# chngdickson/ov2slam

Hardware: AMD Instinct MI355X
Metric: tracked_frames_per_sec (higher is better)
Workload: dtype u8/s16 fixed-point + f32

## Files before the change

### include/ov2slam_hip.h

```cpp
#ifndef OV2SLAM_HIP_H
#define OV2SLAM_HIP_H

#include <stddef.h>
#include <stdint.h>

#ifdef __cplusplus
extern "C" {
#endif

typedef int ov2_status;
enum {
    OV2_OK = 0,
    OV2_ERR_INVALID = -1,
    OV2_ERR_HIP = -2,
    OV2_ERR_NOMEM = -3,
    OV2_ERR_NODEVICE = -4,
    OV2_ERR_UNSUPPORTED = -5
};

typedef struct ov2_ctx ov2_ctx;
typedef struct ov2_images ov2_images;
typedef struct ov2_pyr ov2_pyr;

ov2_status ov2_ctx_create(int device, ov2_ctx **out);
// ... 47 lines not shown
void ov2_pyr_release(ov2_pyr *p);
void ov2_pyr_release_from(ov2_ctx *user, ov2_pyr *p);
int ov2_pyr_batch(const ov2_pyr *p);
int ov2_pyr_nlevels(const ov2_pyr *p);
ov2_status ov2_pyr_level_size(const ov2_pyr *p, int level, int *w, int *h, int *pad);
ov2_status ov2_pyr_download_level(ov2_ctx *ctx, const ov2_pyr *p, int b, int level, uint8_t *img, int16_t *grad);

ov2_status ov2_klt_track_fb(ov2_ctx *ctx, const ov2_pyr *prev, const ov2_pyr *cur, int win, int nlevels,
                            int max_iter, float eps, float err_th, float fb_th, int n, const float *kps_xy,
                            float *priors_xy, uint8_t *status);
ov2_status ov2_klt_track_fb_dev(ov2_ctx *ctx, const ov2_pyr *prev, const ov2_pyr *cur, int win, int nlevels,
                                int max_iter, float eps, float err_th, float fb_th, int n, const float *d_kps_xy,
                                float *d_priors_xy, uint8_t *d_status, const int32_t *d_img_idx,
                                uint32_t *d_iters);

ov2_status ov2_klt_tracking_frame_dev(ov2_ctx *ctx, const ov2_pyr *prev, const ov2_pyr *cur, int win,
                                      int nlevels_full, int max_iter, float eps, float err_th, float fb_th, int n,
                                      const float *d_kps_xy, const float *d_prior_xy, const uint8_t *d_has_prior,
                                      const int32_t *d_img_idx, float *d_out_xy, uint8_t *d_out_status,
                                      int32_t *d_p3p_req , uint32_t *d_iters );

ov2_status ov2_klt_set_lanes(ov2_ctx *ctx, int lanes);
ov2_status ov2_klt_set_stereo_split(ov2_ctx *ctx, int k);

ov2_status ov2_line_min_sad(ov2_ctx *ctx, const ov2_pyr *left, const ov2_pyr *right, int level, int nwinsize, int go_left,
                            int n, const float *pts_xy, float *xprior, float *l1err);
ov2_status ov2_line_min_sad_dev(ov2_ctx *ctx, const ov2_pyr *left, const ov2_pyr *right, int level, int nwinsize,
                                int go_left, int n, const float *d_pts_xy, const int32_t *d_img_idx, float *d_xprior,
                                float *d_l1err);

typedef struct ov2_cam_model {
    double K[4];
    int32_t model;
    int32_t n_coeffs;
    double D[5];
} ov2_cam_model;

ov2_status ov2_stereo_matching(ov2_ctx *ctx, const ov2_pyr *left, const ov2_pyr *right, int win, int nlevels_full,
                               int max_iter, float eps, float err_th, float fb_th, int n, const float *kps_xy,
                               const float *prior_xy, const uint8_t *has_prior, const float *lunpx_xy, int rectified,
                               const double *F_rl, const ov2_cam_model *right_cam, float *out_rxy, uint8_t *out_status);
ov2_status ov2_stereo_matching_dev(ov2_ctx *ctx, const ov2_pyr *left, const ov2_pyr *right, int win, int nlevels_full,
                                   int max_iter, float eps, float err_th, float fb_th, int n, const float *d_kps_xy,
                                   const float *d_prior_xy, const uint8_t *d_has_prior, const int32_t *d_img_idx,
                                   const float *d_lunpx_xy, int rectified, const double *F_rl, const ov2_cam_model *right_cam,
                                   float *d_out_rxy, uint8_t *d_out_status, uint32_t *d_iters);
// ... 487 lines not shown
```

### ov2slam_amd/_lib.py

```python
import ctypes as C
import os

_HERE = os.path.dirname(os.path.abspath(__file__))
LIB_PATH = os.environ.get("OV2SLAM_HIP_LIB") or os.path.join(_HERE, "lib", "libov2hip.so")

vp = C.c_void_p
vpp = C.POINTER(C.c_void_p)
ip = C.POINTER(C.c_int)
fp = C.POINTER(C.c_float)

SIGNATURES = {
    "ov2_ctx_create": (C.c_int, [C.c_int, vpp]),
    "ov2_ctx_create_ex": (C.c_int, [C.c_int, C.c_int, vpp]),
    "ov2_ctx_destroy": (None, [vp]),
    "ov2_last_error": (C.c_char_p, [vp]),
    "ov2_status_string": (C.c_char_p, [C.c_int]),
    "ov2_ctx_synchronize": (C.c_int, [vp]),
    "ov2_ctx_set_kf_overlap": (C.c_int, [vp, C.c_int]),
    "ov2_ctx_set_kf_lazy_join": (C.c_int, [vp, C.c_int]),
    "ov2_ctx_get_kf_lazy_join": (C.c_int, [vp]),
    "ov2_ctx_kf_join_stats": (C.c_int, [vp, C.POINTER(C.c_int64)]),
    "ov2_kf_ranges_independent": (C.c_int, [C.POINTER(C.c_size_t), C.c_int, C.POINTER(C.c_size_t), C.c_int,
                                            C.POINTER(C.c_size_t), C.c_int, C.POINTER(C.c_size_t), C.c_int]),
    "ov2_ctx_set_wave_prio": (C.c_int, [vp, C.c_int]),
# ... 17 lines not shown
    "ov2_memcpy_d2h": (C.c_int, [vp, vp, vp, C.c_size_t]),
    "ov2_memcpy_d2d": (C.c_int, [vp, vp, vp, C.c_size_t]),
    "ov2_images_create": (C.c_int, [vp, C.c_int, C.c_int, C.c_int, vpp]),
    "ov2_images_upload": (C.c_int, [vp, vp, C.c_int, vp, C.c_int]),
    "ov2_images_destroy": (None, [vp]),
    "ov2_pyramid_build": (C.c_int, [vp, vp, C.c_int, C.c_int, C.c_int, C.c_int, C.c_int, C.c_int, C.c_float,
                                    C.c_int, C.c_int, vpp]),
    "ov2_pyramid_build_images": (C.c_int, [vp, vp, C.c_int, C.c_int, C.c_int, C.c_float, C.c_int, C.c_int, vpp]),
    "ov2_pyr_retain": (None, [vp]),
    "ov2_pyr_release": (None, [vp]),
    "ov2_pyr_release_from": (None, [vp, vp]),
    "ov2_pyr_batch": (C.c_int, [vp]),
    "ov2_pyr_nlevels": (C.c_int, [vp]),
    "ov2_pyr_level_size": (C.c_int, [vp, C.c_int, ip, ip, ip]),
    "ov2_pyr_download_level": (C.c_int, [vp, vp, C.c_int, C.c_int, vp, vp]),
    "ov2_klt_track_fb": (C.c_int, [vp, vp, vp, C.c_int, C.c_int, C.c_int, C.c_float, C.c_float, C.c_float,
                                   C.c_int, vp, vp, vp]),
    "ov2_klt_track_fb_dev": (C.c_int, [vp, vp, vp, C.c_int, C.c_int, C.c_int, C.c_float, C.c_float, C.c_float,
                                       C.c_int, vp, vp, vp, vp, vp]),
    "ov2_klt_tracking_frame_dev": (C.c_int, [vp, vp, vp, C.c_int, C.c_int, C.c_int, C.c_float, C.c_float,
                                             C.c_float, C.c_int, vp, vp, vp, vp, vp, vp, vp, vp]),
    "ov2_klt_set_lanes": (C.c_int, [vp, C.c_int]),
    "ov2_klt_set_stereo_split": (C.c_int, [vp, C.c_int]),
    "ov2_line_min_sad": (C.c_int, [vp, vp, vp, C.c_int, C.c_int, C.c_int, C.c_int, vp, vp, vp]),
    "ov2_line_min_sad_dev": (C.c_int, [vp, vp, vp, C.c_int, C.c_int, C.c_int, C.c_int, vp, vp, vp, vp]),
    "ov2_stereo_matching": (C.c_int, [vp, vp, vp, C.c_int, C.c_int, C.c_int, C.c_float, C.c_float, C.c_float, C.c_int,
                                      vp, vp, vp, vp, C.c_int, vp, vp, vp, vp]),
    "ov2_stereo_matching_dev": (C.c_int, [vp, vp, vp, C.c_int, C.c_int, C.c_int, C.c_float, C.c_float, C.c_float, C.c_int,
                                          vp, vp, vp, vp, vp, C.c_int, vp, vp, vp, vp, vp]),
    "ov2_detect_grid": (C.c_int, [vp, vp, C.c_int, C.c_int, C.c_int, C.POINTER(C.c_double), C.c_int, vp, vp, C.c_int, ip, vp]),
    "ov2_detect_grid_batch": (C.c_int, [vp, vp, C.c_int, C.c_int, C.POINTER(C.c_double), ip, vp, vp, C.c_int, ip, vp, C.c_int]),
    "ov2_detect_grid_batch_dev": (C.c_int, [vp, vp, C.c_int, C.c_int, vp, C.c_int, vp, vp, vp, vp, C.c_int, vp, vp, C.c_int]),
    "ov2_fast_detect_batch": (C.c_int, [vp, vp, C.c_int, C.c_int, vp, vp, C.c_int, C.c_int, vp, vp, vp, vp]),
    "ov2_fast_detect_batch_dev": (C.c_int, [vp, vp, C.c_int, C.c_int, C.c_int, vp, vp, C.c_int, C.c_int, vp, vp, vp, vp]),
    "ov2_ba_default_options": (None, [vp, C.c_float]),
    "ov2_ba_solve": (C.c_int, [vp, vp, vp, vp]),
    "ov2_ba_solve_batch": (C.c_int, [vp, C.c_int, vp, vp, vp]),
    "ov2_ba_solve_batch_dev": (C.c_int, [vp, C.c_int, vp, vp, vp]),
    "ov2_pnp_solve_batch_dev": (C.c_int, [vp, C.c_int, vp, vp, vp, vp, vp, vp, C.c_int, C.c_float, C.c_int, C.c_int,
                                          vp, vp, vp, vp]),
    "ov2_map_create": (C.c_int, [vp, C.c_int, C.c_int, C.c_int, vp]),
    "ov2_map_destroy": (None, [vp]),
    "ov2_map_add_keyframe": (C.c_int, [vp, C.c_int, vp, C.c_int, vp, vp, vp, vp, vp]),
    "ov2_map_set_landmarks": (C.c_int, [vp, C.c_int, vp, vp, vp]),
    "ov2_map_set_poses": (C.c_int, [vp, C.c_int, vp, vp]),
    "ov2_map_remove_obs": (C.c_int, [vp, C.c_int, vp, vp]),
# ... 103 lines not shown
```

### ov2slam_amd/csrc/ctx.hip

```cpp
#include "ov2_internal.h"

#include <cstdlib>

ov2_status ov2_set_err(ov2_ctx *ctx, ov2_status s, const char *fmt, ...)
{
    char buf[512];
    va_list ap;
    va_start(ap, fmt);
    vsnprintf(buf, sizeof(buf), fmt, ap);
    va_end(ap);
    if (ctx) {
        std::lock_guard<std::mutex> g(ctx->mu);
        ctx->err = buf;
    }
    return s;
}

extern "C" const char *ov2_status_string(ov2_status s)
{
    switch (s) {
    case OV2_OK: return "ok";
    case OV2_ERR_INVALID: return "invalid argument";
    case OV2_ERR_HIP: return "HIP runtime error";
    case OV2_ERR_NOMEM: return "out of memory";
// ... 91 lines not shown
    if (device < 0 || device >= ndev) return OV2_ERR_INVALID;
    if (hipSetDevice(device) != hipSuccess) return OV2_ERR_HIP;
    uint32_t mask[MAX_MASK_WORDS];
    int mask_words = 0, effective_cus = 0;
    if (n_cus > 0) {
        const int total = device_cus(device);
        if (n_cus >= total || total > 32 * MAX_MASK_WORDS || ov2_cu_mask_build(total, n_cus, layout, mask) != OV2_OK) return OV2_ERR_INVALID;
        mask_words = (total + 31) / 32;
        for (int x = 0; x < OV2_CU_MASK_XCDS; ++x) {
            int bits = 0, own = 0;
            for (int k = x; k < total; k += OV2_CU_MASK_XCDS, ++own) bits += (int)(mask[k >> 5] >> (k & 31) & 1u);
            effective_cus += bits ? bits : own;
        }
    }
    ov2_ctx *c = new ov2_ctx();
    c->device = device;
    c->scratch_dev = nullptr;
    c->scratch_bytes = 0;
    c->tmp_img = nullptr;
    c->ktime_on = false;
    c->wave_prio = high_priority ? OV2_WAVE_PRIO_HIGH : 0;
    c->klt_lanes = 0;
    c->klt_stereo_split = -1;
    c->knn_lanes = 0;
    c->knn_cus = effective_cus;
    c->cu_share = n_cus;
    c->cu_layout = layout;
    c->counts_as_high = false;
    c->lcd_splits = 0;
    c->lcd_calls = 0;
    c->ba_arena = nullptr;
    c->ba_arena_cap = 0;
    c->ba_host = nullptr;
    c->ba_host_cap = 0;
    c->ba_copy_stream = nullptr;
    c->klt_counts[0] = c->klt_counts[1] = nullptr;
    c->klt_counts_words = 0;
    c->klt_counts_cur = 0;
    c->klt_counts_dirty = true;
    c->ba_copy_ev[0] = c->ba_copy_ev[1] = nullptr;
    c->ba_arena2 = nullptr;
    c->ba_arena2_cap = 0;
    c->stage_host = c->stage_dev = nullptr;
    c->stage_cap = 0;
    c->stage_ev = nullptr;
    c->stage_ev_pending = false;
// ... 506 lines not shown
```

### ov2slam_amd/csrc/klt.hip

```cpp
#include <cstdlib>

#include "ov2_internal.h"
#include "ov2_wave.h"

using namespace ov2wave;

namespace {

struct klt_params {
    int win, nlevels, max_iter;
    int wave_prio;
    double eps2;
    float err_th;
    double fb_th;
    float min_eig_thr;
    int rule33;
};

#define W_BITS 14

__device__ __forceinline__ void lk_weights(float a, float b, int &w00, int &w01, int &w10, int &w11)
{
    w00 = (int)__builtin_rintf((1.f - a) * (1.f - b) * (float)(1 << W_BITS));
    w01 = (int)__builtin_rintf(a * (1.f - b) * (float)(1 << W_BITS));
// ... 110 lines not shown
    asm("v_ashrrev_i32_sdwa %0, %2, %1 dst_sel:WORD_1 dst_unused:UNUSED_PRESERVE src0_sel:DWORD src1_sel:DWORD" : "+v"(keep) : "v"(acc), "n"(SH));
    return keep;
}

struct level_ptrs {
    const unsigned char *img;
    const int *grad;
    int istride, gstride, w, h, rows;
    const unsigned char *base;
    unsigned img_o, grad_o;
};

__device__ __forceinline__ level_ptrs level_of(const ov2_pyr_view &v, int l, int b)
{
    level_ptrs p;
    const ov2_level_desc &L = v.lv[l];
    p.img = v.base + L.img_off + L.img_bstride * b;
    p.grad = reinterpret_cast<const int *>(v.base + L.grad_off + L.grad_bstride * b);
    p.istride = L.istride; p.gstride = L.gstride; p.w = L.w; p.h = L.h; p.rows = L.rows;
    p.base = v.base; p.img_o = (unsigned)(L.img_off + L.img_bstride * b); p.grad_o = (unsigned)(L.grad_off + L.grad_bstride * b);
    return p;
}

template <int WIN, int GL>
__device__ __forceinline__ int lk_level(const level_ptrs &I, const level_ptrs &J, int pad, int level, int max_level,
                                        bool run, float kx, float ky, float &nx_io, float &ny_io, int &status,
                                        float &err, const klt_params &P, int sub, unsigned &passes,
                                        unsigned char *lwI, unsigned char *lwJ, unsigned char *lg)
{
    constexpr int GROW = klt_lds<WIN>::GSEG * 4;
    constexpr int OC = WIN < GL ? WIN : GL;
    constexpr int NE = (WIN - OC) * WIN;
    constexpr int NR = (NE + GL - 1) / GL;
    constexpr int NRP = (NR + 1) / 2;
    constexpr int NP = (WIN + 1) / 2;
    const float FLT_SCALE = 1.f / (float)(1 << 20);
    const float half = (float)(WIN - 1) * 0.5f;
    const float lscale = __builtin_ldexpf(1.f, -level);
    float px = kx * lscale, py = ky * lscale;
    float nx, ny;
    if (level == max_level) { nx = nx_io * lscale; ny = ny_io * lscale; }
    else { nx = nx_io * 2.f; ny = ny_io * 2.f; }
    if (run) { nx_io = nx; ny_io = ny; }

    px -= half; py -= half;
    const int ipx = (int)floorf(px), ipy = (int)floorf(py);
    if (run && (ipx < -WIN || ipx >= I.w || ipy < -WIN || ipy >= I.h)) {
        if (level == 0) { status = 0; err = 0.f; }
        run = false;
    }
    if (!__any(run)) return 0;
    if (run) passes += 1u;
    int w00, w01, w10, w11;
    lk_weights(px - (float)ipx, py - (float)ipy, w00, w01, w10, w11);

    const bool col = sub < OC;
    const int sc = col ? sub : 0;
    unsigned Iv2[NP], Ix2[NP], Iy2[NP];
    unsigned IvE[NRP > 0 ? NRP : 1], IxE[NRP > 0 ? NRP : 1], IyE[NRP > 0 ? NRP : 1];
    int eoff[NR > 0 ? NR : 1];
    int sA11 = 0, sA12 = 0, sA22 = 0;
    {
        const unsigned W01 = pack_lo16((unsigned)w00, (unsigned)w01), W23 = pack_lo16((unsigned)w10, (unsigned)w11);
        const int bx0 = run ? (OV2_LM + ipx) : OV2_LM, by = run ? (ipy + pad) : pad;
        {
            const float sx = nx - half, sy = ny - half;
            const int inx0 = (int)floorf(sx), iny0 = (int)floorf(sy);
            const bool in0 = run && !(inx0 < -WIN || inx0 >= J.w || iny0 < -WIN || iny0 >= J.h);
            __syncthreads();
            const int jx0 = OV2_LM + (in0 ? inx0 : 0);
            stage_u8<WIN, GL>(I.img + (size_t)by * I.istride + (bx0 & ~3), I.istride, lwI, sub);
            stage_grad<WIN, GL>(I.grad + (size_t)by * I.gstride + bx0, I.gstride, lg, sub);
            stage_u8<WIN, GL>(J.img + (size_t)((in0 ? iny0 : 0) + pad) * J.istride + (jx0 & ~3), J.istride, lwJ, sub);
            __syncthreads();
        }
        const lds_col ci = lds_col_of(lwI, (bx0 & 3) + sc);
        const int *gp = reinterpret_cast<const int *>(lg) + sc;
        unsigned T = spread_u8x2(lds_pair(ci, 0));
        unsigned GX, GY;
        {
            const unsigned g0 = (unsigned)gp[0], g1 = (unsigned)gp[1];
            GX = pack_lo16(g0, g1); GY = pack_hi16(g0, g1);
        }
        const bool on = run && col;
        unsigned piv = 0, pix = 0, piy = 0;
#pragma unroll
        for (int y = 0; y < WIN; ++y) {
            gp += GROW;
            const unsigned B = spread_u8x2(lds_pair(ci, y + 1));
            const unsigned h0 = (unsigned)gp[0], h1 = (unsigned)gp[1];
            const unsigned HX = pack_lo16(h0, h1), HY = pack_hi16(h0, h1);
            const unsigned iv = (unsigned)dot2(B, W23, dot2k(T, W01, 1 << (W_BITS - 5 - 1))) >> (W_BITS - 5);
            int ix = dot2(HX, W23, dot2k(GX, W01, 1 << (W_BITS - 1))) >> W_BITS;
            int iy = dot2(HY, W23, dot2k(GY, W01, 1 << (W_BITS - 1))) >> W_BITS;
            if (y & 1) {
                Iv2[y >> 1] = pack_lo16(piv, iv); Ix2[y >> 1] = pack_lo16(pix, (unsigned)ix); Iy2[y >> 1] = pack_lo16(piy, (unsigned)iy);
            } else if (y == WIN - 1) {
                Iv2[y >> 1] = iv; Ix2[y >> 1] = (unsigned)ix & 0xffffu; Iy2[y >> 1] = (unsigned)iy & 0xffffu;
            } else {
                piv = iv; pix = (unsigned)ix; piy = (unsigned)iy;
            }
            T = B; GX = HX; GY = HY;
        }
        {
            const unsigned onm = on ? 0xffffffffu : 0u;
#pragma unroll
            for (int q = 0; q < NP; ++q) {
                Ix2[q] &= onm; Iy2[q] &= onm;
                sA11 = dot2(Ix2[q], Ix2[q], sA11); sA12 = dot2(Ix2[q], Iy2[q], sA12); sA22 = dot2(Iy2[q], Iy2[q], sA22);
            }
        }
#pragma unroll
        for (int r = 0; r < NR; ++r) {
            const int e = sub + GL * r;
            const bool ev = e < NE;
            const int ec = ev ? e : 0;
            const int ecol = OC + ec / WIN, erow = ec - (ec / WIN) * WIN;
            eoff[r] = erow * 16 + ecol;
            const lds_col ce = lds_col_of(lwI + erow * 16, (bx0 & 3) + ecol);
            const int *gpe = reinterpret_cast<const int *>(lg) + erow * GROW + ecol;
            const unsigned T0 = spread_u8x2(lds_pair(ce, 0)), T1 = spread_u8x2(lds_pair(ce, 1));
            const unsigned g0 = (unsigned)gpe[0], g1 = (unsigned)gpe[1];
            const unsigned h0 = (unsigned)gpe[GROW], h1 = (unsigned)gpe[GROW + 1];
            const unsigned iv = (unsigned)dot2(T1, W23, dot2k(T0, W01, 1 << (W_BITS - 5 - 1))) >> (W_BITS - 5);
            int ix = dot2(pack_lo16(h0, h1), W23, dot2k(pack_lo16(g0, g1), W01, 1 << (W_BITS - 1))) >> W_BITS;
// ... 122 lines not shown

template <int GL>
struct klt_map {
    static constexpr int KPW = 64 / GL;
    static __device__ __forceinline__ int slot(int tid) { return tid / GL; }
    static __device__ __forceinline__ int sub(int tid) { return tid & (GL - 1); }
    static __device__ __forceinline__ bool lane_ok(int) { return true; }
};
template <>
struct klt_map<3> {
    static constexpr int KPW = 21;
    static __device__ __forceinline__ int slot(int tid) { return min((tid * 171) >> 9, KPW - 1); }
    static __device__ __forceinline__ int sub(int tid) { return tid == 63 ? 0 : tid - 3 * ((tid * 171) >> 9); }
    static __device__ __forceinline__ bool lane_ok(int tid) { return tid != 63; }
};

template <int WIN, int GL>
struct klt_smem {
    static constexpr int BYTES = (64 / GL) * (2 * klt_lds<WIN>::WB + klt_lds<WIN>::GB);
};
template <int WIN>
struct klt_smem<WIN, 3> {
    static constexpr int BYTES = klt_map<3>::KPW * klt3::RSZ;
};

__device__ __forceinline__ int sum3_i32(int v, int c)
{
    const int t1 = v + dpp_i32<0x138>(v);
    const int t = v + dpp_i32<0x138>(t1);
    const int u1 = dpp_mov_i32<0x130>(t), u2 = dpp_mov_i32<0x130>(u1);
    return c == 2 ? t : (c == 1 ? u1 : u2);
}
__device__ __forceinline__ double sum3_f64(double v, int c)
{
    const double s1 = dpp_f64<0x138>(v), s2 = dpp_f64<0x138>(s1);
    const double t = (v + s1) + s2;
    const double u1 = dpp_f64<0x130>(t), u2 = dpp_f64<0x130>(u1);
    return c == 2 ? t : (c == 1 ? u1 : u2);
}

__device__ __forceinline__ unsigned klt3_pair_sel(unsigned k) { return 0x0c010c00u + k * 0x00010001u; }

__device__ __forceinline__ void klt3_region_origin(const level_ptrs &J, int pad, int inx, int iny, int &rr0, int &cc0)
{
    rr0 = min(max(iny + pad - klt3::ROW_MARGIN, 0), J.rows - klt3::RROWS);
    cc0 = min(max((OV2_LM + inx - klt3::COL_LEAD) & ~(klt3::COL_ALIGN - 1), 0), J.istride - klt3::RBYTES);
// ... 251 lines not shown
            b1 = (float)sum3_i32(pb1, c) * FLT_SCALE;
            b2 = (float)sum3_i32(pb2, c) * FLT_SCALE;
        } else {
            b1 = (float)sum3_f64((double)pb1, c) * FLT_SCALE;
            b2 = (float)sum3_f64((double)pb2, c) * FLT_SCALE;
        }
        const float dx = (A12 * b2 - A22 * b1) * D;
        const float dy = (A12 * b1 - A11 * b2) * D;
        if (run) {
            ++iters;
            nx += dx; ny += dy;
            nx_io = nx + half; ny_io = ny + half;
            if ((double)dx * dx + (double)dy * dy <= P.eps2) run = false;
            else if (j > 0 && fabsf(dx + pdx) <= 0.01f && fabsf(dy + pdy) <= 0.01f) {
                nx_io -= dx * 0.5f; ny_io -= dy * 0.5f;
                run = false;
            }
            pdx = dx; pdy = dy;
        }
    }
    return iters;
}

template <int WIN, int GL>
__device__ __forceinline__ int lk_pass(const level_ptrs &I, const level_ptrs &J, int pad, int level, int max_level, bool run,
                                       float kx, float ky, float &nx_io, float &ny_io, int &status, float &err,
                                       const klt_params &P, int sub, bool lane_ok, unsigned &passes, unsigned char *smem, int slot)
{
    if constexpr (GL == 3) {
        return lk_level3<WIN>(I, J, pad, level, max_level, run, kx, ky, nx_io, ny_io, status, err, P, sub, lane_ok, passes,
                              smem + slot * klt3::RSZ);
    } else {
        constexpr int KPW = 64 / GL, WB = klt_lds<WIN>::WB, GB = klt_lds<WIN>::GB;
        return lk_level<WIN, GL>(I, J, pad, level, max_level, run, kx, ky, nx_io, ny_io, status, err, P, sub, passes,
                                 smem + slot * WB, smem + KPW * WB + slot * WB, smem + 2 * KPW * WB + slot * GB);
    }
}

struct __attribute__((aligned(16))) klt_handover { float fx, fy, err; unsigned work; };

template <int WIN, int GL>
__device__ __forceinline__ int fb_track(const ov2_pyr_view &pv, const ov2_pyr_view &cv, int b, bool act, float kx,
                                          float ky, float &fx, float &fy, const klt_params &P, int nlevels, int sub,
                                          bool lane_ok, unsigned &work, unsigned char *smem, int slot,
                                          int l_hi, int l_lo, float err0, unsigned work0, float &err_out)
{
    int status = 1;
    float err = err0;
    unsigned it = work0 & 0xffffu, passes = work0 >> 16;
    for (int l = l_hi; l >= l_lo; --l) {
        const level_ptrs I = level_of(pv, l, b), J = level_of(cv, l, b);
        it += lk_pass<WIN, GL>(I, J, pv.pad, l, nlevels, act, kx, ky, fx, fy, status, err, P, sub, lane_ok, passes, smem, slot);
    }
    if (l_lo > 0) {
        work = it | (passes << 16);
        err_out = err;
        return 0;
    }
    const int W0 = cv.lv[0].w, H0 = cv.lv[0].h;
    int ok = act && status && !(err > P.err_th) &&
             (1.f <= fx && fx < (float)W0 - 1.f && 1.f <= fy && fy < (float)H0 - 1.f);
    int st2 = 1;
    float e2 = 0.f, bx = kx, by = ky;
    {
        const level_ptrs I = level_of(cv, 0, b), J = level_of(pv, 0, b);
        it += lk_pass<WIN, GL>(I, J, cv.pad, 0, 0, ok != 0, fx, fy, bx, by, st2, e2, P, sub, lane_ok, passes, smem, slot);
    }
    if (ok) {
        if (!st2) ok = 0;
        else {
            const float dx = kx - bx, dy = ky - by;
            const double nrm = __dsqrt_rn((double)dx * dx + (double)dy * dy);
            if (nrm > P.fb_th) ok = 0;
        }
    }
    work = it | (passes << 16);
    return ok;
}

template <int WIN, int GL>
__device__ __forceinline__ int fb_track(const ov2_pyr_view &pv, const ov2_pyr_view &cv, int b, bool act, float kx,
                                          float ky, float &fx, float &fy, const klt_params &P, int nlevels, int sub,
                                          bool lane_ok, unsigned &work, unsigned char *smem, int slot)
{
    float err;
    return fb_track<WIN, GL>(pv, cv, b, act, kx, ky, fx, fy, P, nlevels, sub, lane_ok, work, smem, slot, nlevels, 0, 0.f, 0u, err);
}

#define KLT_GL8_MIN_KPS 65536
// ... 133 lines not shown
    const int total = is_a ? total_a : total_b;
    if (g * KLT_KPW >= total) return;
    ov2wave::set_wave_prio(P.wave_prio);
    const int slot = M::slot((int)threadIdx.x), sub = M::sub((int)threadIdx.x), idx = g * KLT_KPW + slot;
    const bool lane_ok = M::lane_ok((int)threadIdx.x);
    const bool act = idx < total && lane_ok;
    const int i = (is_a ? list_a : list_b)[idx < total ? idx : total - 1];
    const float2 kp = kps[i];
    const int b = img_idx ? img_idx[i] : 0;
    float2 pr = (is_a || !P.rule33) ? prior[i] : kp;
    unsigned work = 0;
    const int nl = is_a ? min(1, pv.nlevels - 1) : P.nlevels;
    const bool upper = SPLIT && !is_a;
    float err;
    const int ok = fb_track<WIN, KLT_GL>(pv, cv, b, act, kp.x, kp.y, pr.x, pr.y, P, nl, sub, lane_ok, work, smem, slot, nl,
                                         upper ? split_k + 1 : 0, 0.f, 0u, err);
    if (upper) {
        if (act && sub == 0) hand[i] = klt_handover{pr.x, pr.y, err, work};
        return;
    }
    klt_stage1_finish(act && sub == 0, is_a, i, b, n, ok, pr, work, out_xy, out_status, counts, iters, cnt, list_c);
}

template <int WIN, int KLT_GL>
__global__ __launch_bounds__(64) __attribute__((amdgpu_waves_per_eu(KLT_WAVES(WIN, KLT_GL)))) void klt_stage2_kernel(ov2_pyr_view pv, ov2_pyr_view cv, klt_params P, int n,
                                                        const float2 *__restrict__ kps,
                                                        const int *__restrict__ img_idx, float2 *__restrict__ out_xy,
                                                        unsigned char *__restrict__ out_status,
                                                        const unsigned *__restrict__ counts, int *__restrict__ p3p_req,
                                                        unsigned *__restrict__ iters, const int *__restrict__ list_c,
                                                        const unsigned *__restrict__ cnt, int batch,
                                                        unsigned *__restrict__ next_counts, int next_words,
                                                        const int *__restrict__ list_b, int b_word,
                                                        const float2 *__restrict__ prior,
                                                        int split_k ,
                                                        const klt_handover *__restrict__ hand)
{
    __shared__ __attribute__((aligned(16))) unsigned char smem[klt_smem<WIN, KLT_GL>::BYTES];
    using M = klt_map<KLT_GL>;
    constexpr int KLT_KPW = M::KPW;
    const int slot = M::slot((int)threadIdx.x), sub = M::sub((int)threadIdx.x);
    const bool lane_ok = M::lane_ok((int)threadIdx.x);
    for (int q = blockIdx.x * 64 + threadIdx.x; q < next_words; q += gridDim.x * 64) next_counts[q] = 0u;
    auto tally = [&](int b, int &n3, int &good) {
        n3 = 0; good = 0;
        if constexpr (KLT_GL == 3) {
            for (int q = sub; q < 64; q += 3) {
                const unsigned cw = counts[64 * b + q];
                n3 += (int)(cw & 0xffffu); good += (int)(cw >> 16);
            }
            n3 = sum3_i32(n3, sub); good = sum3_i32(good, sub);
        } else {
            for (int q = 0; q < 64 / KLT_GL; ++q) {
                const unsigned cw = counts[64 * b + sub * (64 / KLT_GL) + q];
                n3 += (int)(cw & 0xffffu); good += (int)(cw >> 16);
            }
            n3 = row_sum_i32<KLT_GL>(n3); good = row_sum_i32<KLT_GL>(good);
        }
    };
    if (p3p_req && P.rule33) {
        for (int b0 = blockIdx.x * KLT_KPW; b0 < batch; b0 += gridDim.x * KLT_KPW) {
            const int b = b0 + slot;
            int n3, good;
            tally(min(b, batch - 1), n3, good);
            if (b < batch && lane_ok && sub == 0 && n3 > 0 && (double)good < 0.33 * (double)n3) p3p_req[b] = 1;
        }
    }
    const int total_b = (int)cnt[b_word], total_c = (int)cnt[2];
    const bool b_first = split_k < 0 || !KLT_SPLIT_C_FIRST;
    const int groups_1 = ((b_first ? total_b : total_c) + KLT_KPW - 1) / KLT_KPW;
    const bool first = (int)blockIdx.x < groups_1;
    const bool is_b = first == b_first;
    const int g = first ? (int)blockIdx.x : (int)blockIdx.x - groups_1;
    const int total = is_b ? total_b : total_c;
    if (g * KLT_KPW >= total) return;
    ov2wave::set_wave_prio(P.wave_prio);
    const int idx = g * KLT_KPW + slot;
    const bool act = idx < total && lane_ok;
    const int i = (is_b ? list_b : list_c)[idx < total ? idx : total - 1];
    const int b = img_idx ? img_idx[i] : 0;
    const float2 kp = kps[i];
    float2 pr;
    int l_hi = P.nlevels;
    float err0 = 0.f;
    unsigned work0 = 0;
    if (is_b) {
        if (split_k >= 0) {
            const klt_handover hr = hand[i];
            pr = make_float2(hr.fx, hr.fy);
            err0 = hr.err; work0 = hr.work; l_hi = split_k;
        } else {
            pr = prior[i];
        }
    } else {
        int n3, good;
        tally(b, n3, good);
        const bool drop = P.rule33 && n3 > 0 && (double)good < 0.33 * (double)n3;
        pr = drop ? kp : out_xy[i];
    }
    unsigned work = 0;
    float err;
    const int ok = fb_track<WIN, KLT_GL>(pv, cv, b, act, kp.x, kp.y, pr.x, pr.y, P, P.nlevels, sub, lane_ok, work, smem, slot,
                                         l_hi, 0, err0, work0, err);
    if (act && sub == 0) {
        out_xy[i] = pr;
        out_status[i] = (unsigned char)ok;
        if (iters) iters[n + i] = work;
    }
}

int klt_lanes_for(const ov2_ctx *c, int n, int win, const ov2_pyr *a, const ov2_pyr *b)
{
    static const int env = [] { const char *e = getenv("OV2_KLT_LANES"); return e ? atoi(e) : 0; }();
    const int forced = c->klt_lanes ? c->klt_lanes : env;
    const bool fits32 = a->buf->bytes < (1ull << 32) && b->buf->bytes < (1ull << 32);
    if (forced == 8 || forced == 16 || (forced == 3 && win == 9 && fits32)) return forced;
    if (win == 9 && fits32) return 3;
    return n >= KLT_GL8_MIN_KPS ? 8 : 16;
}

ov2_status make_params(ov2_ctx *c, const ov2_pyr *prev, const ov2_pyr *cur, int win, int nlevels, int max_iter,
                       float eps, float err_th, float fb_th, klt_params *P)
{
    if (!prev || !cur) return ov2_set_err(c, OV2_ERR_INVALID, "null pyramid");
    const ov2_pyr_view &a = prev->buf->view, &b = cur->buf->view;
    if (a.nlevels != b.nlevels || a.pad != b.pad || a.batch != b.batch || a.lv[0].w != b.lv[0].w ||
        a.lv[0].h != b.lv[0].h)
        return ov2_set_err(c, OV2_ERR_INVALID, "prev/cur pyramids differ in geometry");
    if (win < 3 || win > 11 || (win & 1) == 0 || win > a.pad)
        return ov2_set_err(c, OV2_ERR_INVALID, "win=%d unsupported (odd, 3..11, <= pyramid pad %d)", win, a.pad);
    if (nlevels < 0) return ov2_set_err(c, OV2_ERR_INVALID, "nlevels < 0");
    if (a.nlevels < nlevels + 1) nlevels = a.nlevels - 1;
    P->win = win;
    P->wave_prio = c->wave_prio;
    P->nlevels = nlevels;
    P->max_iter = max_iter < 0 ? 0 : (max_iter > 100 ? 100 : max_iter);
    double e = (double)eps;
    if (e < 0.) e = 0.;
    if (e > 10.) e = 10.;
    P->eps2 = e * e;
    P->err_th = err_th;
    P->fb_th = (double)fb_th;
    P->min_eig_thr = 1e-4f;
    P->rule33 = 1;
    return OV2_OK;
}

}

extern "C" ov2_status ov2_klt_set_lanes(ov2_ctx *c, int lanes)
{
    if (!c) return OV2_ERR_INVALID;
    if (lanes != 0 && lanes != 3 && lanes != 8 && lanes != 16) return ov2_set_err(c, OV2_ERR_INVALID, "lanes per keypoint: 0 (auto), 3, 8 or 16");
    c->klt_lanes = lanes;
    return OV2_OK;
}

extern "C" ov2_status ov2_klt_set_stereo_split(ov2_ctx *c, int k)
{
    if (!c) return OV2_ERR_INVALID;
    c->klt_stereo_split = k < 0 ? -1 : k;
    return OV2_OK;
}

extern "C" ov2_status ov2_klt_track_fb_dev(ov2_ctx *c, const ov2_pyr *prev, const ov2_pyr *cur, int win, int nlevels,
                                           int max_iter, float eps, float err_th, float fb_th, int n,
                                           const float *d_kps, float *d_priors, uint8_t *d_status,
                                           const int32_t *d_img_idx, uint32_t *d_iters)
{
    if (!c) return OV2_ERR_INVALID;
    if (n == 0) return OV2_OK;
    if (n < 0 || !d_kps || !d_priors || !d_status) return ov2_set_err(c, OV2_ERR_INVALID, "null/negative argument");
    klt_params P;
    ov2_status s = make_params(c, prev, cur, win, nlevels, max_iter, eps, err_th, fb_th, &P);
    if (s != OV2_OK) return s;
    OV2_HIP(c, hipSetDevice(c->device));
    if ((s = ov2_pyr_wait_ready(c, prev)) != OV2_OK || (s = ov2_pyr_wait_ready(c, cur)) != OV2_OK) return s;
    const int lanes = klt_lanes_for(c, n, win, prev, cur);
// ... 93 lines not shown
    c->klt_counts_dirty = true;
    void *scr = nullptr;
    const size_t lists_bytes = (3 * (size_t)n * sizeof(int) + 255) / 256 * 256;
    s = ov2_scratch(c, lists_bytes + (size_t)n * sizeof(klt_handover) + 256, &scr);
    if (s != OV2_OK) return s;
    unsigned *counts = c->klt_counts[c->klt_counts_cur], *live_cnt = counts + (size_t)B * 64;
    unsigned *next_counts = c->klt_counts[c->klt_counts_cur ^ 1];
    const int next_words = (int)c->klt_counts_words;
    int *list_a = (int *)scr, *list_b = list_a + n, *list_c = list_b + n;
    const size_t N = (size_t)n;
    const ov2_byte_range kf_rd[4] = {ov2_range(d_kps, 8 * N), ov2_range(d_prior, 8 * N), ov2_range(d_has_prior, N), ov2_range(d_img_idx, 4 * N)};
    const ov2_byte_range kf_wr[4] = {ov2_range(d_out_xy, 8 * N), ov2_range(d_out_status, N), ov2_range(d_p3p_req, sizeof(int32_t) * (size_t)B),
                                     ov2_range(d_iters, 8 * N)};
    const hipStream_t ms = ov2_kf_stream_for(c, true, kf_rd, 4, kf_wr, 4);
    if (c->kf.want_stereo_ev) {
        OV2_HIP(c, hipEventRecord(c->kf.fork, c->stream.h));
        c->kf.want_stereo_ev = false;
    }
    const dim3 cgrid((n + KLT_COMPACT_KPWG - 1) / KLT_COMPACT_KPWG);
    const int want_k = c->klt_stereo_split < 0 ? KLT_STEREO_SPLIT_DEFAULT : c->klt_stereo_split;
    const int split_k = (!P.rule33 && want_k < P.nlevels) ? want_k : -1;
    const int b_word1 = (P.rule33 || split_k >= 0) ? 1 : 3, b_word2 = P.rule33 ? 3 : 1;
    klt_handover *hand = reinterpret_cast<klt_handover *>((char *)scr + lists_bytes);
#define KLT_STAGES_GL(W, G)                                                                                     \
    do {                                                                                                        \
         \
        const dim3 tgrid((n + klt_map<G>::KPW - 1) / klt_map<G>::KPW + 2);                                      \
        OV2_LAUNCH_ON(c, OV2_K_DETECT + 4, ms, klt_compact_kernel, cgrid, dim3(256), 0, ms, n, d_has_prior,     \
                   d_iters, list_a, list_b, live_cnt, d_p3p_req, B, P.wave_prio);                               \
        if (split_k >= 0)                                                                                       \
            OV2_LAUNCH_ON(c, OV2_K_KLT_STAGE1, ms, (klt_stage1_kernel<W, G, true>), tgrid, dim3(64), 0, ms,     \
                       prev->buf->view, cur->buf->view, P, n, reinterpret_cast<const float2 *>(d_kps),          \
                       reinterpret_cast<const float2 *>(d_prior), d_img_idx, reinterpret_cast<float2 *>(d_out_xy), \
                       d_out_status, counts, d_iters, list_a, list_b, live_cnt, list_c, b_word1, split_k, hand); \
        else                                                                                                    \
            OV2_LAUNCH_ON(c, OV2_K_KLT_STAGE1, ms, (klt_stage1_kernel<W, G, false>), tgrid, dim3(64), 0, ms,    \
                       prev->buf->view, cur->buf->view, P, n, reinterpret_cast<const float2 *>(d_kps),          \
                       reinterpret_cast<const float2 *>(d_prior), d_img_idx, reinterpret_cast<float2 *>(d_out_xy), \
                       d_out_status, counts, d_iters, list_a, list_b, live_cnt, list_c, b_word1, split_k, hand); \
        OV2_LAUNCH_ON(c, OV2_K_KLT_STAGE2, ms, (klt_stage2_kernel<W, G>), tgrid, dim3(64), 0, ms,               \
                   prev->buf->view, cur->buf->view, P, n, reinterpret_cast<const float2 *>(d_kps), d_img_idx,   \
                   reinterpret_cast<float2 *>(d_out_xy), d_out_status, counts, d_p3p_req, d_iters, list_c,      \
                   live_cnt, B, next_counts, next_words, list_b, b_word2,                                       \
                   reinterpret_cast<const float2 *>(d_prior), split_k, hand);                                   \
    } while (0)
#define KLT_STAGES(W)                                                                                           \
    do {                                                                                                        \
        if (lanes == 8) KLT_STAGES_GL(W, 8);                                                                       \
        else KLT_STAGES_GL(W, 16);                                                                              \
    } while (0)
    switch (win) {
    case 3: KLT_STAGES(3); break;
    case 5: KLT_STAGES(5); break;
    case 7: KLT_STAGES(7); break;
    case 9:
        if (lanes == 3) KLT_STAGES_GL(9, 3);
        else KLT_STAGES(9);
        break;
    default: KLT_STAGES(11); break;
    }
#undef KLT_STAGES
#undef KLT_STAGES_GL
    OV2_HIP(c, hipGetLastError());
    c->klt_counts_cur ^= 1;
    c->klt_counts_dirty = false;
    return OV2_OK;
}
// ... 1 lines not shown
```

### ov2slam_amd/csrc/ov2_internal.h

```cpp
#pragma once
#include <hip/hip_runtime.h>

#include <atomic>
#include <cstdarg>
#include <cstdio>
#include <cstring>
#include <mutex>
#include <string>
#include <vector>

#include "../../include/ov2slam_hip.h"

#define OV2_MAX_LEVELS 8
#define OV2_LM 16

struct ov2_level_desc {
    int w, h;
    int istride;
    int gstride;
    int rows;
    size_t img_off;
    size_t grad_off;
    size_t img_bstride;
    size_t grad_bstride;
// ... 140 lines not shown
    std::string err;
    void *scratch_dev;
    size_t scratch_bytes;
    ov2_images *tmp_img;
    void *ba_arena;
    size_t ba_arena_cap;
    void *stage_host, *stage_dev;
    size_t stage_cap;
    hipEvent_t stage_ev;
    bool stage_ev_pending;
    void *ba_arena2;
    size_t ba_arena2_cap;
    void *ba_host;
    size_t ba_host_cap;
    unsigned *klt_counts[2];
    size_t klt_counts_words;
    int klt_counts_cur;
    bool klt_counts_dirty;
    hipStream_t ba_copy_stream;
    hipEvent_t ba_copy_ev[2];
    int wave_prio;
    int klt_lanes;
    int klt_stereo_split;
    int knn_lanes;
    int knn_cus;
    int cu_share, cu_layout;
    bool counts_as_high;
    int lcd_splits;
    long long lcd_calls;
    std::vector<struct ov2_lcd_table *> lcd_tables;
    bool ktime_on;
    std::vector<ov2_ktime_rec> ktime_recs;
    std::vector<hipEvent_t> ktime_free;
};

struct ov2_images {
    ov2_ctx *ctx;
    int batch, w, h;
    int stride;
    size_t bstride;
    unsigned char *base;
};

struct ov2_pyr {
    std::atomic<int> refs;
    ov2_ctx *ctx;
// ... 43 lines not shown
```

### ov2slam_amd/frontend.py

```python
import ctypes as C

import numpy as np

from . import _lib


WAVE_PRIO_HIGH = 2


CU_LAYOUT_SPREAD, CU_LAYOUT_PACKED = 0, 1
CU_MASK_XCDS = 8


def cu_mask_build(total_cus, n_cus, layout=CU_LAYOUT_SPREAD):
    out = (C.c_uint32 * ((int(total_cus) + 31) // 32 if total_cus > 0 else 1))()
    st = _lib.load().ov2_cu_mask_build(int(total_cus), int(n_cus), int(layout), out)
    if st != 0:
        raise _lib.Ov2Error(f"ov2_cu_mask_build({total_cus}, {n_cus}, {layout}): status {st}")
    return np.array(out, np.uint32)


def _check(ctx_handle, status):
    if status != 0:
        lib = _lib.load()
# ... 11 lines not shown
        else:
            st = self.lib.ov2_ctx_create_cu(device, int(bool(high_priority)), int(cu_share), int(cu_layout), C.byref(h))
            if st == -1:
                raise _lib.Ov2Error(f"ov2_ctx_create_cu(device={device}, high_priority={bool(high_priority)}, n_cus={cu_share}, "
                                    f"layout={cu_layout}): {self.lib.ov2_status_string(st).decode()}")
        if st != 0:
            raise _lib.Ov2Error(f"ov2_ctx_create(device={device}): {self.lib.ov2_status_string(st).decode()} -- "
                                "an MI355X/gfx950 device is required, there is no CPU fallback")
        self.h = h

    def close(self):
        if getattr(self, "h", None):
            self.lib.ov2_ctx_destroy(self.h)
            self.h = None

    def __del__(self):
        self.close()

    def set_klt_lanes(self, lanes):
        _check(self.h, self.lib.ov2_klt_set_lanes(self.h, int(lanes)))

    def set_stereo_split(self, k):
        _check(self.h, self.lib.ov2_klt_set_stereo_split(self.h, int(k)))

    def set_knn_lanes(self, lanes):
        _check(self.h, self.lib.ov2_knn_set_lanes(self.h, int(lanes)))

    def set_kf_overlap(self, on):
        _check(self.h, self.lib.ov2_ctx_set_kf_overlap(self.h, int(bool(on))))

    def set_wave_prio(self, level):
        _check(self.h, self.lib.ov2_ctx_set_wave_prio(self.h, int(level)))

    def get_wave_prio(self):
        return int(self.lib.ov2_ctx_get_wave_prio(self.h))

    def get_cu_share(self):
        return int(self.lib.ov2_ctx_get_cu_share(self.h))

    def get_cu_mask(self, words):
        out = (C.c_uint32 * int(words))()
        _check(self.h, self.lib.ov2_ctx_get_cu_mask(self.h, int(words), out))
        return np.array(out, np.uint32)

    def set_kf_lazy_join(self, on):
        _check(self.h, self.lib.ov2_ctx_set_kf_lazy_join(self.h, int(bool(on))))
# ... 353 lines not shown
```

Measured before the change: 311,000.

## Retrack list-C keypoints with 16 lanes and in-kernel Scharr gradients

In the stage-2 KLT kernel, when the 3-lane path is used for 9x9 windows, the list-C re-tracked keypoints now run on a 16-lanes-per-keypoint layout. Those blocks loop over chunks, and the block count is capped by the grid slots left after list B. This path computes Scharr derivatives inside the kernel from staged image rows rather than loading precomputed gradients, which trades gradient memory traffic for extra packed ALU work. Default selection uses 16 lanes for tracking (rule33) and 3 for stereo, with a context setter and env override. It risks load imbalance from capping the groups and small fixed-point differences at image borders.

```diff
diff --git a/include/ov2slam_hip.h b/include/ov2slam_hip.h
--- a/include/ov2slam_hip.h
+++ b/include/ov2slam_hip.h
@@ -93,6 +93,8 @@
 
 ov2_status ov2_klt_set_lanes(ov2_ctx *ctx, int lanes);
 ov2_status ov2_klt_set_stereo_split(ov2_ctx *ctx, int k);
+ov2_status ov2_klt_set_retrack_lanes(ov2_ctx *ctx, int lanes);
+int ov2_klt_retrack_groups(int n, int total_b, int total_c, int *groups, int *chunks_per_group);
 
 ov2_status ov2_line_min_sad(ov2_ctx *ctx, const ov2_pyr *left, const ov2_pyr *right, int level, int nwinsize, int go_left,
                             int n, const float *pts_xy, float *xprior, float *l1err);
diff --git a/ov2slam_amd/_lib.py b/ov2slam_amd/_lib.py
--- a/ov2slam_amd/_lib.py
+++ b/ov2slam_amd/_lib.py
@@ -63,6 +63,8 @@
                                              C.c_float, C.c_int, vp, vp, vp, vp, vp, vp, vp, vp]),
     "ov2_klt_set_lanes": (C.c_int, [vp, C.c_int]),
     "ov2_klt_set_stereo_split": (C.c_int, [vp, C.c_int]),
+    "ov2_klt_set_retrack_lanes": (C.c_int, [vp, C.c_int]),
+    "ov2_klt_retrack_groups": (C.c_int, [C.c_int, C.c_int, C.c_int, C.POINTER(C.c_int), C.POINTER(C.c_int)]),
     "ov2_line_min_sad": (C.c_int, [vp, vp, vp, C.c_int, C.c_int, C.c_int, C.c_int, vp, vp, vp]),
     "ov2_line_min_sad_dev": (C.c_int, [vp, vp, vp, C.c_int, C.c_int, C.c_int, C.c_int, vp, vp, vp, vp]),
     "ov2_stereo_matching": (C.c_int, [vp, vp, vp, C.c_int, C.c_int, C.c_int, C.c_float, C.c_float, C.c_float, C.c_int,
diff --git a/ov2slam_amd/csrc/ctx.hip b/ov2slam_amd/csrc/ctx.hip
--- a/ov2slam_amd/csrc/ctx.hip
+++ b/ov2slam_amd/csrc/ctx.hip
@@ -137,6 +137,7 @@
     c->wave_prio = high_priority ? OV2_WAVE_PRIO_HIGH : 0;
     c->klt_lanes = 0;
     c->klt_stereo_split = -1;
+    c->klt_retrack_lanes = 0;
     c->knn_lanes = 0;
     c->knn_cus = effective_cus;
     c->cu_share = n_cus;
diff --git a/ov2slam_amd/csrc/klt.hip b/ov2slam_amd/csrc/klt.hip
--- a/ov2slam_amd/csrc/klt.hip
+++ b/ov2slam_amd/csrc/klt.hip
@@ -156,7 +156,7 @@
     return p;
 }
 
-template <int WIN, int GL>
+template <int WIN, int GL, bool SCHARR = false>
 __device__ __forceinline__ int lk_level(const level_ptrs &I, const level_ptrs &J, int pad, int level, int max_level,
                                         bool run, float kx, float ky, float &nx_io, float &ny_io, int &status,
                                         float &err, const klt_params &P, int sub, unsigned &passes,
@@ -197,44 +197,90 @@
     {
         const unsigned W01 = pack_lo16((unsigned)w00, (unsigned)w01), W23 = pack_lo16((unsigned)w10, (unsigned)w11);
         const int bx0 = run ? (OV2_LM + ipx) : OV2_LM, by = run ? (ipy + pad) : pad;
+        const bool on = run && col;
         {
             const float sx = nx - half, sy = ny - half;
             const int inx0 = (int)floorf(sx), iny0 = (int)floorf(sy);
             const bool in0 = run && !(inx0 < -WIN || inx0 >= J.w || iny0 < -WIN || iny0 >= J.h);
             __syncthreads();
             const int jx0 = OV2_LM + (in0 ? inx0 : 0);
-            stage_u8<WIN, GL>(I.img + (size_t)by * I.istride + (bx0 & ~3), I.istride, lwI, sub);
-            stage_grad<WIN, GL>(I.grad + (size_t)by * I.gstride + bx0, I.gstride, lg, sub);
+            if constexpr (SCHARR) {
+                if (sub < WIN + 3) {
+                    const int dr = sub == 0 ? (by > 0 ? -1 : 0) : (sub == WIN + 2 ? (by + WIN + 1 < I.rows ? WIN + 1 : WIN) : sub - 1);
+                    *reinterpret_cast<uint4 *>(lwI + sub * 16) = ld_b128(I.img + (size_t)(by + dr) * I.istride + ((bx0 - 1) & ~3));
+                }
+            } else {
+                stage_u8<WIN, GL>(I.img + (size_t)by * I.istride + (bx0 & ~3), I.istride, lwI, sub);
+                stage_grad<WIN, GL>(I.grad + (size_t)by * I.gstride + bx0, I.gstride, lg, sub);
+            }
             stage_u8<WIN, GL>(J.img + (size_t)((in0 ? iny0 : 0) + pad) * J.istride + (jx0 & ~3), J.istride, lwJ, sub);
             __syncthreads();
         }
-        const lds_col ci = lds_col_of(lwI, (bx0 & 3) + sc);
-        const int *gp = reinterpret_cast<const int *>(lg) + sc;
-        unsigned T = spread_u8x2(lds_pair(ci, 0));
-        unsigned GX, GY;
-        {
-            const unsigned g0 = (unsigned)gp[0], g1 = (unsigned)gp[1];
-            GX = pack_lo16(g0, g1); GY = pack_hi16(g0, g1);
-        }
-        const bool on = run && col;
         unsigned piv = 0, pix = 0, piy = 0;
-#pragma unroll
-        for (int y = 0; y < WIN; ++y) {
-            gp += GROW;
-            const unsigned B = spread_u8x2(lds_pair(ci, y + 1));
-            const unsigned h0 = (unsigned)gp[0], h1 = (unsigned)gp[1];
-            const unsigned HX = pack_lo16(h0, h1), HY = pack_hi16(h0, h1);
-            const unsigned iv = (unsigned)dot2(B, W23, dot2k(T, W01, 1 << (W_BITS - 5 - 1))) >> (W_BITS - 5);
-            int ix = dot2(HX, W23, dot2k(GX, W01, 1 << (W_BITS - 1))) >> W_BITS;
-            int iy = dot2(HY, W23, dot2k(GY, W01, 1 << (W_BITS - 1))) >> W_BITS;
-            if (y & 1) {
-                Iv2[y >> 1] = pack_lo16(piv, iv); Ix2[y >> 1] = pack_lo16(pix, (unsigned)ix); Iy2[y >> 1] = pack_lo16(piy, (unsigned)iy);
-            } else if (y == WIN - 1) {
-                Iv2[y >> 1] = iv; Ix2[y >> 1] = (unsigned)ix & 0xffffu; Iy2[y >> 1] = (unsigned)iy & 0xffffu;
-            } else {
-                piv = iv; pix = (unsigned)ix; piy = (unsigned)iy;
-            }
-            T = B; GX = HX; GY = HY;
+        if constexpr (SCHARR) {
+            static_assert(!SCHARR || (WIN == 9 && GL == 16), "in-kernel derivatives: 9 x 9 windows, lane = window column");
+            const lds_col ct = lds_col_of(lwI, ((bx0 - 1) & 3) + sc);
+            const int x0 = ipx + sc;
+            const unsigned wlim = on ? (unsigned)I.w : 0u, hlim = on ? (unsigned)I.h : 0u;
+            const unsigned cm = ((unsigned)x0 < wlim ? 0xffffu : 0u) | ((unsigned)(x0 + 1) < wlim ? 0xffff0000u : 0u);
+            const unsigned W01g = W01 & cm, W23g = W23 & cm;
+            unsigned Pm0 = 0, Pm1 = 0, Hd0 = 0, Hd1 = 0, Hd2 = 0, Sm0 = 0, Sm1 = 0, Sm2 = 0, GXp = 0, GYp = 0;
+#pragma unroll
+            for (int p = 0; p < WIN + 3; ++p) {
+                const unsigned q4 = lds_pair(ct, p);
+                const unsigned P0 = __builtin_amdgcn_perm(0u, q4, 0x0c010c00u), P1 = __builtin_amdgcn_perm(0u, q4, 0x0c020c01u),
+                               P2 = __builtin_amdgcn_perm(0u, q4, 0x0c030c02u);
+                Hd0 = Hd1; Hd1 = Hd2; Sm0 = Sm1; Sm1 = Sm2;
+                Hd2 = pk_sub16(P2, P0);
+                Sm2 = pk_mad16(P1, 10u, pk_mul16(pk_add16(P0, P2), 3u));
+                if (p >= 2) {
+                    const unsigned rm = (unsigned)(ipy + p - 2) < hlim ? 0xffffffffu : 0u;
+                    const unsigned GX = pk_mad16(Hd1, 10u, pk_mul16(pk_add16(Hd0, Hd2), 3u)) & rm;
+                    const unsigned GY = pk_sub16(Sm2, Sm0) & rm;
+                    if (p >= 3) {
+                        const int y = p - 3;
+                        const unsigned iv = (unsigned)dot2(Pm1, W23, dot2k(Pm0, W01, 1 << (W_BITS - 5 - 1))) >> (W_BITS - 5);
+                        const int ix = dot2(GX, W23g, dot2k(GXp, W01g, 1 << (W_BITS - 1))) >> W_BITS;
+                        const int iy = dot2(GY, W23g, dot2k(GYp, W01g, 1 << (W_BITS - 1))) >> W_BITS;
+                        if (y & 1) {
+                            Iv2[y >> 1] = pack_lo16(piv, iv); Ix2[y >> 1] = pack_lo16(pix, (unsigned)ix); Iy2[y >> 1] = pack_lo16(piy, (unsigned)iy);
+                        } else if (y == WIN - 1) {
+                            Iv2[y >> 1] = iv; Ix2[y >> 1] = (unsigned)ix & 0xffffu; Iy2[y >> 1] = (unsigned)iy & 0xffffu;
+                        } else {
+                            piv = iv; pix = (unsigned)ix; piy = (unsigned)iy;
+                        }
+                    }
+                    GXp = GX; GYp = GY;
+                }
+                Pm0 = Pm1; Pm1 = P1;
+            }
+        } else {
+            const lds_col ci = lds_col_of(lwI, (bx0 & 3) + sc);
+            const int *gp = reinterpret_cast<const int *>(lg) + sc;
+            unsigned T = spread_u8x2(lds_pair(ci, 0));
+            unsigned GX, GY;
+            {
+                const unsigned g0 = (unsigned)gp[0], g1 = (unsigned)gp[1];
+                GX = pack_lo16(g0, g1); GY = pack_hi16(g0, g1);
+            }
+#pragma unroll
+            for (int y = 0; y < WIN; ++y) {
+                gp += GROW;
+                const unsigned B = spread_u8x2(lds_pair(ci, y + 1));
+                const unsigned h0 = (unsigned)gp[0], h1 = (unsigned)gp[1];
+                const unsigned HX = pack_lo16(h0, h1), HY = pack_hi16(h0, h1);
+                const unsigned iv = (unsigned)dot2(B, W23, dot2k(T, W01, 1 << (W_BITS - 5 - 1))) >> (W_BITS - 5);
+                int ix = dot2(HX, W23, dot2k(GX, W01, 1 << (W_BITS - 1))) >> W_BITS;
+                int iy = dot2(HY, W23, dot2k(GY, W01, 1 << (W_BITS - 1))) >> W_BITS;
+                if (y & 1) {
+                    Iv2[y >> 1] = pack_lo16(piv, iv); Ix2[y >> 1] = pack_lo16(pix, (unsigned)ix); Iy2[y >> 1] = pack_lo16(piy, (unsigned)iy);
+                } else if (y == WIN - 1) {
+                    Iv2[y >> 1] = iv; Ix2[y >> 1] = (unsigned)ix & 0xffffu; Iy2[y >> 1] = (unsigned)iy & 0xffffu;
+                } else {
+                    piv = iv; pix = (unsigned)ix; piy = (unsigned)iy;
+                }
+                T = B; GX = HX; GY = HY;
+            }
         }
         {
             const unsigned onm = on ? 0xffffffffu : 0u;
@@ -403,6 +449,11 @@
 template <int WIN>
 struct klt_smem<WIN, 3> {
     static constexpr int BYTES = klt_map<3>::KPW * klt3::RSZ;
+};
+template <int WIN, int GL>
+struct klt_scharr_smem {
+    static constexpr int TB = (WIN + 3) * 16 + 16;
+    static constexpr int BYTES = (64 / GL) * (TB + klt_lds<WIN>::WB);
 };
 
 __device__ __forceinline__ int sum3_i32(int v, int c)
@@ -700,7 +751,7 @@
     return iters;
 }
 
-template <int WIN, int GL>
+template <int WIN, int GL, bool SCHARR = false>
 __device__ __forceinline__ int lk_pass(const level_ptrs &I, const level_ptrs &J, int pad, int level, int max_level, bool run,
                                        float kx, float ky, float &nx_io, float &ny_io, int &status, float &err,
                                        const klt_params &P, int sub, bool lane_ok, unsigned &passes, unsigned char *smem, int slot)
@@ -708,6 +759,10 @@
     if constexpr (GL == 3) {
         return lk_level3<WIN>(I, J, pad, level, max_level, run, kx, ky, nx_io, ny_io, status, err, P, sub, lane_ok, passes,
                               smem + slot * klt3::RSZ);
+    } else if constexpr (SCHARR) {
+        constexpr int KPW = 64 / GL, TB = klt_scharr_smem<WIN, GL>::TB, WB = klt_lds<WIN>::WB;
+        return lk_level<WIN, GL, true>(I, J, pad, level, max_level, run, kx, ky, nx_io, ny_io, status, err, P, sub, passes,
+                                       smem + slot * TB, smem + KPW * TB + slot * WB, nullptr);
     } else {
         constexpr int KPW = 64 / GL, WB = klt_lds<WIN>::WB, GB = klt_lds<WIN>::GB;
         return lk_level<WIN, GL>(I, J, pad, level, max_level, run, kx, ky, nx_io, ny_io, status, err, P, sub, passes,
@@ -717,7 +772,7 @@
 
 struct __attribute__((aligned(16))) klt_handover { float fx, fy, err; unsigned work; };
 
-template <int WIN, int GL>
+template <int WIN, int GL, bool SCHARR = false>
 __device__ __forceinline__ int fb_track(const ov2_pyr_view &pv, const ov2_pyr_view &cv, int b, bool act, float kx,
                                           float ky, float &fx, float &fy, const klt_params &P, int nlevels, int sub,
                                           bool lane_ok, unsigned &work, unsigned char *smem, int slot,
@@ -728,7 +783,7 @@
     unsigned it = work0 & 0xffffu, passes = work0 >> 16;
     for (int l = l_hi; l >= l_lo; --l) {
         const level_ptrs I = level_of(pv, l, b), J = level_of(cv, l, b);
-        it += lk_pass<WIN, GL>(I, J, pv.pad, l, nlevels, act, kx, ky, fx, fy, status, err, P, sub, lane_ok, passes, smem, slot);
+        it += lk_pass<WIN, GL, SCHARR>(I, J, pv.pad, l, nlevels, act, kx, ky, fx, fy, status, err, P, sub, lane_ok, passes, smem, slot);
     }
     if (l_lo > 0) {
         work = it | (passes << 16);
@@ -742,7 +797,7 @@
     float e2 = 0.f, bx = kx, by = ky;
     {
         const level_ptrs I = level_of(cv, 0, b), J = level_of(pv, 0, b);
-        it += lk_pass<WIN, GL>(I, J, cv.pad, 0, 0, ok != 0, fx, fy, bx, by, st2, e2, P, sub, lane_ok, passes, smem, slot);
+        it += lk_pass<WIN, GL, SCHARR>(I, J, cv.pad, 0, 0, ok != 0, fx, fy, bx, by, st2, e2, P, sub, lane_ok, passes, smem, slot);
     }
     if (ok) {
         if (!st2) ok = 0;
@@ -922,6 +977,12 @@
     klt_stage1_finish(act && sub == 0, is_a, i, b, n, ok, pr, work, out_xy, out_status, counts, iters, cnt, list_c);
 }
 
+__host__ __device__ inline int klt_retrack_groups(int grid, int groups_b, int total_c)
+{
+    const int chunks = (total_c + 3) / 4, room = grid - groups_b;
+    return chunks < room ? chunks : room;
+}
+
 template <int WIN, int KLT_GL>
 __global__ __launch_bounds__(64) __attribute__((amdgpu_waves_per_eu(KLT_WAVES(WIN, KLT_GL)))) void klt_stage2_kernel(ov2_pyr_view pv, ov2_pyr_view cv, klt_params P, int n,
                                                         const float2 *__restrict__ kps,
@@ -934,9 +995,11 @@
                                                         const int *__restrict__ list_b, int b_word,
                                                         const float2 *__restrict__ prior,
                                                         int split_k ,
-                                                        const klt_handover *__restrict__ hand)
+                                                        const klt_handover *__restrict__ hand,
+                                                        int retrack16 )
 {
     __shared__ __attribute__((aligned(16))) unsigned char smem[klt_smem<WIN, KLT_GL>::BYTES];
+    static_assert(!(WIN == 9 && KLT_GL == 3) || klt_scharr_smem<9, 16>::BYTES <= klt_smem<WIN, KLT_GL>::BYTES, "list C's 16-lane layout shares the block");
     using M = klt_map<KLT_GL>;
     constexpr int KLT_KPW = M::KPW;
     const int slot = M::slot((int)threadIdx.x), sub = M::sub((int)threadIdx.x);
@@ -958,6 +1021,14 @@
             n3 = row_sum_i32<KLT_GL>(n3); good = row_sum_i32<KLT_GL>(good);
         }
     };
+    auto tally16 = [&](int b, int &n3, int &good, int sub16) {
+        n3 = 0; good = 0;
+        for (int q = 0; q < 4; ++q) {
+            const unsigned cw = counts[64 * b + sub16 * 4 + q];
+            n3 += (int)(cw & 0xffffu); good += (int)(cw >> 16);
+        }
+        n3 = row_sum_i32<16>(n3); good = row_sum_i32<16>(good);
+    };
     if (p3p_req && P.rule33) {
         for (int b0 = blockIdx.x * KLT_KPW; b0 < batch; b0 += gridDim.x * KLT_KPW) {
             const int b = b0 + slot;
@@ -968,10 +1039,42 @@
     }
     const int total_b = (int)cnt[b_word], total_c = (int)cnt[2];
     const bool b_first = split_k < 0 || !KLT_SPLIT_C_FIRST;
-    const int groups_1 = ((b_first ? total_b : total_c) + KLT_KPW - 1) / KLT_KPW;
+    const bool c16 = WIN == 9 && KLT_GL == 3 && retrack16 != 0;
+    const int groups_b = (total_b + KLT_KPW - 1) / KLT_KPW;
+    const int groups_c = c16 ? klt_retrack_groups((int)gridDim.x, groups_b, total_c) : (total_c + KLT_KPW - 1) / KLT_KPW;
+    const int groups_1 = b_first ? groups_b : groups_c;
     const bool first = (int)blockIdx.x < groups_1;
     const bool is_b = first == b_first;
     const int g = first ? (int)blockIdx.x : (int)blockIdx.x - groups_1;
+    if constexpr (WIN == 9 && KLT_GL == 3) {
+        if (c16 && !is_b) {
+            if (g >= groups_c) return;
+            ov2wave::set_wave_prio(P.wave_prio);
+            using M16 = klt_map<16>;
+            const int slot16 = M16::slot((int)threadIdx.x), sub16 = M16::sub((int)threadIdx.x);
+            for (int ch = g; ch * M16::KPW < total_c; ch += groups_c) {
+                const int idx = ch * M16::KPW + slot16;
+                const bool act = idx < total_c;
+                const int i = list_c[act ? idx : total_c - 1];
+                const int b = img_idx ? img_idx[i] : 0;
+                const float2 kp = kps[i];
+                int n3, good;
+                tally16(b, n3, good, sub16);
+                const bool drop = P.rule33 && n3 > 0 && (double)good < 0.33 * (double)n3;
+                float2 pr = drop ? kp : out_xy[i];
+                unsigned work = 0;
+                float err;
+                const int ok = fb_track<9, 16, true>(pv, cv, b, act, kp.x, kp.y, pr.x, pr.y, P, P.nlevels, sub16, true, work, smem,
+                                                     slot16, P.nlevels, 0, 0.f, 0u, err);
+                if (act && sub16 == 0) {
+                    out_xy[i] = pr;
+                    out_status[i] = (unsigned char)ok;
+                    if (iters) iters[n + i] = work;
+                }
+            }
+            return;
+        }
+    }
     const int total = is_b ? total_b : total_c;
     if (g * KLT_KPW >= total) return;
     ov2wave::set_wave_prio(P.wave_prio);
@@ -1017,6 +1120,20 @@
     if (forced == 8 || forced == 16 || (forced == 3 && win == 9 && fits32)) return forced;
     if (win == 9 && fits32) return 3;
     return n >= KLT_GL8_MIN_KPS ? 8 : 16;
+}
+
+#ifndef KLT_RETRACK_LANES_TRACK
+#define KLT_RETRACK_LANES_TRACK 16
+#endif
+#ifndef KLT_RETRACK_LANES_STEREO
+#define KLT_RETRACK_LANES_STEREO 3
+#endif
+int klt_retrack_lanes_for(const ov2_ctx *c, int lanes, int rule33)
+{
+    static const int env = [] { const char *e = getenv("OV2_KLT_RETRACK_LANES"); return e ? atoi(e) : 0; }();
+    if (lanes != 3) return lanes;
+    const int want = c->klt_retrack_lanes ? c->klt_retrack_lanes : env;
+    return (want == 3 || want == 16) ? want : (rule33 ? KLT_RETRACK_LANES_TRACK : KLT_RETRACK_LANES_STEREO);
 }
 
 ov2_status make_params(ov2_ctx *c, const ov2_pyr *prev, const ov2_pyr *cur, int win, int nlevels, int max_iter,
@@ -1054,6 +1171,25 @@
     if (lanes != 0 && lanes != 3 && lanes != 8 && lanes != 16) return ov2_set_err(c, OV2_ERR_INVALID, "lanes per keypoint: 0 (auto), 3, 8 or 16");
     c->klt_lanes = lanes;
     return OV2_OK;
+}
+
+extern "C" ov2_status ov2_klt_set_retrack_lanes(ov2_ctx *c, int lanes)
+{
+    if (!c) return OV2_ERR_INVALID;
+    if (lanes != 0 && lanes != 3 && lanes != 16) return ov2_set_err(c, OV2_ERR_INVALID, "lanes per re-tracked keypoint: 0 (built-in), 3 or 16");
+    c->klt_retrack_lanes = lanes;
+    return OV2_OK;
+}
+
+extern "C" int ov2_klt_retrack_groups(int n, int total_b, int total_c, int *groups, int *chunks_per_group)
+{
+    if (n <= 0 || total_b < 0 || total_c < 0 || (long long)total_b + total_c > n || !groups || !chunks_per_group) return -1;
+    constexpr int KPW = klt_map<3>::KPW;
+    const int grid = (n + KPW - 1) / KPW + 2, groups_b = (total_b + KPW - 1) / KPW;
+    const int g = klt_retrack_groups(grid, groups_b, total_c), chunks = (total_c + 3) / 4;
+    *groups = g;
+    *chunks_per_group = g ? (chunks + g - 1) / g : 0;
+    return 0;
 }
 
 extern "C" ov2_status ov2_klt_set_stereo_split(ov2_ctx *c, int k)
@@ -1193,6 +1329,7 @@
     const int split_k = (!P.rule33 && want_k < P.nlevels) ? want_k : -1;
     const int b_word1 = (P.rule33 || split_k >= 0) ? 1 : 3, b_word2 = P.rule33 ? 3 : 1;
     klt_handover *hand = reinterpret_cast<klt_handover *>((char *)scr + lists_bytes);
+    const int retrack16 = klt_retrack_lanes_for(c, lanes, P.rule33) == 16 ? 1 : 0;
 #define KLT_STAGES_GL(W, G)                                                                                     \
     do {                                                                                                        \
          \
@@ -1213,7 +1350,7 @@
                    prev->buf->view, cur->buf->view, P, n, reinterpret_cast<const float2 *>(d_kps), d_img_idx,   \
                    reinterpret_cast<float2 *>(d_out_xy), d_out_status, counts, d_p3p_req, d_iters, list_c,      \
                    live_cnt, B, next_counts, next_words, list_b, b_word2,                                       \
-                   reinterpret_cast<const float2 *>(d_prior), split_k, hand);                                   \
+                   reinterpret_cast<const float2 *>(d_prior), split_k, hand, retrack16);                        \
     } while (0)
 #define KLT_STAGES(W)                                                                                           \
     do {                                                                                                        \
diff --git a/ov2slam_amd/csrc/ov2_internal.h b/ov2slam_amd/csrc/ov2_internal.h
--- a/ov2slam_amd/csrc/ov2_internal.h
+++ b/ov2slam_amd/csrc/ov2_internal.h
@@ -186,6 +186,7 @@
     int wave_prio;
     int klt_lanes;
     int klt_stereo_split;
+    int klt_retrack_lanes;
     int knn_lanes;
     int knn_cus;
     int cu_share, cu_layout;
diff --git a/ov2slam_amd/frontend.py b/ov2slam_amd/frontend.py
--- a/ov2slam_amd/frontend.py
+++ b/ov2slam_amd/frontend.py
@@ -57,6 +57,9 @@
 
     def set_stereo_split(self, k):
         _check(self.h, self.lib.ov2_klt_set_stereo_split(self.h, int(k)))
+
+    def set_retrack_lanes(self, lanes):
+        _check(self.h, self.lib.ov2_klt_set_retrack_lanes(self.h, int(lanes)))
 
     def set_knn_lanes(self, lanes):
         _check(self.h, self.lib.ov2_knn_set_lanes(self.h, int(lanes)))
```

After: 311,000. About the same (-0.0%).
